# envoy/ksql

Measured on AMD Instinct MI355X. Metric: records/sec, windowed GROUP BY (COUNT(*) TUMBLING 5 s GROUP BY card_number HAVING > 3), higher is better.
Workload: dtype int64

## Files before the change

### ksql_amd/csrc/khip_agg_c1.hip

```cpp
#include <algorithm>
#include <cstdio>
#include <type_traits>
#include <vector>

#include "khip_part.hpp"

namespace khip {

constexpr int C1_TILE = 65536;
constexpr int C1_NT = 512;
constexpr int C1_CH = 8192;
template <class T>
__device__ __forceinline__ T c1_ld(const T* p) {
  return *p;
}
constexpr int C1_SEGMAX = 512;
constexpr int C1_SEGB = 7;
constexpr int C1_SEGOF = 512;
constexpr uint32_t C1_SENT = 0x80000000u;

__device__ __forceinline__ int bits_of(uint64_t v) { return v ? 64 - __clzll((long long)v) : 0; }

__device__ __forceinline__ int64_t ci_ld(const int64_t* ci, int k) {
  const uint64_t v = (uint64_t)__hip_atomic_load(&ci[k], __ATOMIC_RELAXED, __HIP_MEMORY_SCOPE_AGENT);
// ... 295 lines not shown
    ts4[3] = t_ok ? 1 : 0;
  }
}

__global__ __launch_bounds__(256) void k_c1_krange(const int64_t* __restrict__ keys, int64_t stride, int64_t n,
                                                   long long* __restrict__ out) {
  int64_t mx = INT64_MIN, mxn = INT64_MIN;
  for (int64_t i = blockIdx.x * (int64_t)blockDim.x + threadIdx.x; i < n; i += (int64_t)gridDim.x * blockDim.x) {
    const int64_t k = keys[i * stride];
    mx = k > mx ? k : mx;
    mxn = ~k > mxn ? ~k : mxn;
  }
  for (int off = 32; off > 0; off >>= 1) {
    const int64_t a = __shfl_xor(mx, off, 64), b = __shfl_xor(mxn, off, 64);
    mx = a > mx ? a : mx;
    mxn = b > mxn ? b : mxn;
  }
  if ((threadIdx.x & 63) == 0) {
    atomicMax(&out[0], (long long)mxn);
    atomicMax(&out[1], (long long)mx);
  }
}

__global__ __launch_bounds__(1024) void k_c1_runpos(const uint32_t* __restrict__ ttot, int64_t nT,
                                                    uint32_t* __restrict__ tbase) {
  __shared__ uint32_t wsum[16];
  const int lane = threadIdx.x & 63, wave = threadIdx.x >> 6;
  const uint32_t* in = ttot + (int64_t)blockIdx.x * nT;
  uint32_t* out = tbase + (int64_t)blockIdx.x * (nT + 1);
  uint32_t carry = 0u;
  for (int64_t t0 = 0; t0 < nT; t0 += 1024) {
    const int64_t t = t0 + threadIdx.x;
    const uint32_t c = t < nT ? in[t] : 0u;
    uint32_t incl = c;
    for (int off = 1; off < 64; off <<= 1) {
      const uint32_t y = __shfl_up(incl, off, 64);
      if (lane >= off) incl += y;
    }
    if (lane == 63) wsum[wave] = incl;
    __syncthreads();
    uint32_t before = 0u, tot = 0u;
#pragma unroll
    for (int k = 0; k < 16; k++) {
      before += k < wave ? wsum[k] : 0u;
      tot += wsum[k];
    }
    if (t < nT) out[t] = carry + before + incl - c;
    carry += tot;
    __syncthreads();
  }
  if (threadIdx.x == 0) out[nT] = carry;
}

__global__ __launch_bounds__(256) void k_c1_chunks(const int* __restrict__ cstart, int B,
                                                   const uint32_t* __restrict__ tbase, const uint16_t* __restrict__ rloc,
                                                   int64_t nT, int sh, int ch, const int64_t* __restrict__ ci,
                                                   uint32_t* __restrict__ cinfo) {
  if (ci_ld(ci, CI_GATE) == 0) return;
  const int w = blockIdx.x * blockDim.x + threadIdx.x;
  if (w >= (int)ci_ld(ci, CI_NCHUNK)) return;
  int a = 0, e = B;
  while (e - a > 1) {
    const int m = (a + e) >> 1;
    if (cstart[m] <= w) a = m;
    else e = m;
  }
  const int b = a;
  const int64_t nSt = nT << sh, spt = (int64_t)1 << sh;
  const uint32_t* tb = tbase + (int64_t)b * (nT + 1);
  const uint16_t* rl = rloc + (int64_t)b * nSt;
  const int64_t lo = (int64_t)(w - cstart[b]) * ch, blen = (int64_t)tb[nT];
  const int64_t hi = blen - lo < ch ? blen : lo + ch;
  int64_t t0 = 0, e0 = nT, t1 = 0, e1 = nT;
  while (e0 - t0 > 1 || e1 - t1 > 1) {
    const int64_t m0 = (t0 + e0) >> 1, m1 = (t1 + e1) >> 1;
    const int64_t p0 = (int64_t)tb[m0], p1 = (int64_t)tb[m1];
    if (e0 - t0 > 1) {
      if (p0 <= lo) t0 = m0;
      else e0 = m0;
    }
    if (e1 - t1 > 1) {
      if (p1 < hi) t1 = m1;
      else e1 = m1;
    }
  }
  const int64_t b0 = (int64_t)tb[t0], b1 = (int64_t)tb[t1];
  int64_t sa = t0 << sh, sl = t1 << sh;
  for (int64_t half = spt >> 1; half > 0; half >>= 1) {
    const int64_t q0 = b0 + (int64_t)rl[sa + half], q1 = b1 + (int64_t)rl[sl + half];
    if (q0 <= lo) sa += half;
    if (q1 < hi) sl += half;
  }
  cinfo[2 * w] = (uint32_t)sa;
  cinfo[2 * w + 1] = (uint32_t)(sl + 1 - sa);
}

__device__ __forceinline__ void chunk_map(const uint32_t* __restrict__ tb, const uint16_t* __restrict__ rl,
                                          const uint16_t* __restrict__ ro, int64_t nSt, int sh,
                                          const uint32_t* __restrict__ cinfo, int w, int64_t S, int64_t lo, int len,
                                          uint32_t* map) {
  const int64_t s0 = cinfo[2 * w];
  const int R = (int)cinfo[2 * w + 1];
  for (int k = threadIdx.x; k < R; k += blockDim.x) {
    const int64_t s = s0 + k, p = run_pos(tb, rl, nSt, sh, s), pe = run_pos(tb, rl, nSt, sh, s + 1);
    const int64_t a = p > lo ? p : lo, e = pe < lo + len ? pe : lo + len;
    const uint32_t src = (uint32_t)(s * S + (int64_t)ro[s] + (a - p));
    for (int64_t x = a; x < e; x++) map[x - lo] = src + (uint32_t)(x - a);
  }
  __syncthreads();
}

__global__ __launch_bounds__(1024) void k_c1_check(
    const int64_t* __restrict__ tilestat, const int64_t* __restrict__ tpart, int64_t nT, int64_t size, int64_t adv,
    FastDiv fd, int64_t grace, int64_t close0, int fresh, int log2B, int log2P, int wide, int ch, int kbmax, int pbits,
    const uint32_t* __restrict__ tbase, int64_t* __restrict__ bb, int* __restrict__ cstart,
    int64_t* __restrict__ ci, int64_t* __restrict__ stream_time, int64_t* __restrict__ res,
    unsigned long long* __restrict__ ctr, unsigned long long* __restrict__ closed_ctr, unsigned long long closed_n) {
  __shared__ int64_t wmx[16];
  __shared__ int64_t red[2][16];
  __shared__ unsigned long long lsum[T_NPART];
  __shared__ int lslow;
  __shared__ int64_t wtot[8];
  __shared__ int wnch[8], wmxc[8];
  const int lane = threadIdx.x & 63, wave = threadIdx.x >> 6;
  if (threadIdx.x == 0) lslow = 0;
  if (threadIdx.x < T_NPART) lsum[threadIdx.x] = 0ULL;
  const int B = 1 << log2B;
  const uint32_t btot = (int)threadIdx.x < B ? tbase[(int64_t)threadIdx.x * (nT + 1) + nT] : 0u;
  const int64_t st0 = *stream_time;
  const int64_t K = (nT + 1023) / 1024;
  const int64_t g0 = threadIdx.x * K, g1 = g0 + K < nT ? g0 + K : nT;
  int64_t m = -1;
  for (int64_t g = g0; g < g1; g++) m = tilestat[4 * g] > m ? tilestat[4 * g] : m;
  const int64_t incl = wave_incl_max(m);
  if (lane == 63) wmx[wave] = incl;
  __syncthreads();
  int64_t pre = st0;
  for (int w = 0; w < wave; w++) pre = wmx[w] > pre ? wmx[w] : pre;
  const int64_t excl = __shfl_up(incl, 1, 64);
  int64_t run = lane == 0 ? pre : (excl > pre ? excl : pre);
  int64_t gmn = INT64_MAX, gmx = -1;
  int64_t tsum[T_NPART] = {};
  bool slow = false;
  for (int64_t g = g0; g < g1; g++) {
    const int64_t* t4 = tilestat + 4 * g;
    const int64_t mx = t4[0], mn = t4[1];
    if (mn != INT64_MAX) {
      slow |= t4[3] == 0 || run > t4[2];
      gmn = mn < gmn ? mn : gmn;
    }
    run = mx > run ? mx : run;
    gmx = mx > gmx ? mx : gmx;
#pragma unroll
    for (int k = 0; k < T_NPART; k++) tsum[k] += tpart[g * T_NPART + k];
  }
  if (slow) lslow = 1;
  for (int off = 32; off > 0; off >>= 1) {
    const int64_t a = __shfl_xor(gmn, off, 64), b = __shfl_xor(gmx, off, 64);
    gmn = a < gmn ? a : gmn;
    gmx = b > gmx ? b : gmx;
  }
#pragma unroll
// ... 60 lines not shown
           (int)lslow, mxc, (long)kmin, (long)kmax, (long)gmn, (long)gmx, (long)ci[CI_T0], (long)st0, (long)nT);
#endif
  const uint64_t krange = kmax >= kmin ? (uint64_t)kmax - (uint64_t)kmin : 0;
  const bool fits = !wide && !kfail && krange < ((1ULL << kbmax) - 1);
  const int64_t kb = ci_ld(ci, CI_KBASE);
  ci[CI_FITS] = fits ? 1 : 0;
  ci[CI_REASON] = ok && !wide && kfail ? 2 : (ok && !wide && !fits ? 1 : 0);
  ci[CI_KMINC] = kmin;
  ci[CI_KSHIFT] = (int64_t)((uint64_t)kmin - (uint64_t)kb);
  ok = ok && (wide || fits);
  int64_t lo = INT64_MAX, hi = INT64_MIN;
  if (gmx >= 0) {
    const int64_t l = gmn - size + adv;
    lo = (int64_t)fast_udiv((uint64_t)(l > 0 ? l : 0), fd);
    hi = (int64_t)fast_udiv((uint64_t)gmx, fd);
  }
  if (!fresh) {
    int64_t rlo = res[0];
    const int64_t rhi = res[1];
    if (close0 != INT64_MIN && rlo != INT64_MAX) {
      const int64_t c = close0 - size;
      const int64_t lb = c >= 0 ? (int64_t)fast_udiv((uint64_t)c, fd) + 1 : 0;
      rlo = rlo > lb ? rlo : lb;
    }
    lo = rlo < lo ? rlo : lo;
    hi = rhi > hi ? rhi : hi;
  }
  const bool none = lo > hi;
  if (none) lo = hi = 0;
  ok = ok && (uint64_t)(hi - lo) < (wide ? ((uint64_t)1 << log2P) - 1 : (pbits ? 0x7FFFFFFEull : 0xFFFFFFFEull));
  const int wbits = bits_of((uint64_t)(hi - lo)), kbits = bits_of(krange);
  ci[CI_GATE] = ok ? 1 : 0;
  if (!ok) return;
  ci[CI_WBASE] = lo;
  ci[CI_WHI] = hi - lo;
  ci[CI_WBITS] = wbits;
  ci[CI_KBITS] = kbits;
  ci[CI_KRANGE] = (int64_t)krange;
  ci[CI_ID32] = !wide && kbits + wbits + pbits <= 31 ? 1 : 0;
  ci[CI_WIDE] = wide;
  ci[CI_TMIN] = gmx >= 0 ? gmn : 0;
  ci[CI_TMAX] = gmx;
  ci[CI_NCHUNK] = acc;
  *stream_time = gmx > st0 ? gmx : st0;
  res[0] = none ? INT64_MAX : lo;
  res[1] = none ? INT64_MIN : hi;
  ctr[CTR_ADDED] = ctr[CTR_FAILED] = ctr[CTR_NEED] = 0ULL;
  for (int k = 0; k < T_NPART; k++) ctr[CTR_TILE + k] = lsum[k];
  if (closed_ctr) *closed_ctr = closed_n;
}

template <int U, int NT, bool WIDE>
__global__ __launch_bounds__(NT) __attribute__((amdgpu_waves_per_eu(4))) void k_c1_refine(
    const uint64_t* __restrict__ srcA, const int64_t* __restrict__ bb, const int* __restrict__ cstart, int log2B,
    int log2P, int fbits, uint64_t* __restrict__ srec, uint16_t* __restrict__ seg, const int64_t* __restrict__ ci,
    const uint32_t* __restrict__ srcAT, uint32_t* __restrict__ srecT, const uint32_t* __restrict__ tbase,
    const uint16_t* __restrict__ rloc, const uint16_t* __restrict__ roff, int64_t nT, int sh, int64_t S,
    const uint32_t* __restrict__ cinfo) {
  if (ci_ld(ci, CI_GATE) == 0) return;
  const int w = blockIdx.x;
  if (w >= (int)ci_ld(ci, CI_NCHUNK)) return;
  extern __shared__ __attribute__((aligned(16))) char smem[];
  __shared__ int lb, lnv;
  __shared__ int wsum[NT / 64];
  static_assert(U * NT == C1_CH, "refine chunk");
  const int F = 1 << fbits, B = 1 << log2B;
  uint32_t* cnt = (uint32_t*)smem;
  uint32_t* sbase = cnt + F;
  uint64_t* stage = (uint64_t*)(smem + (size_t)F * 8);
  for (int f = threadIdx.x; f < F; f += NT) cnt[f] = 0u;
  if (threadIdx.x == 0) lb = -1;
  __syncthreads();
  for (int b = threadIdx.x; b < B; b += NT)
    if (cstart[b] <= w && w < cstart[b + 1]) lb = b;
  __syncthreads();
  const int b = lb;
  if (b < 0) return;
  const int64_t lo = bb[b] + (int64_t)(w - cstart[b]) * C1_CH;
  const int64_t bend = bb[b + 1];
  const int len = (int)(bend - lo < C1_CH ? bend - lo : C1_CH);
  const int64_t kmin = ci_ld(ci, CI_KMINC);
  const uint64_t kshift = WIDE ? 0 : (uint64_t)ci_ld(ci, CI_KSHIFT) << 32;
  const int shift = 64 - log2P;
  const int64_t nSt = nT << sh;
  chunk_map(tbase + (int64_t)b * (nT + 1), rloc + (int64_t)b * nSt, roff + (int64_t)b * nSt, nSt, sh, cinfo, w, S,
            lo - bb[b], len, (uint32_t*)stage);
  uint64_t r[U];
  uint32_t f[U], rank[U], t32[U];
#pragma unroll
  for (int u = 0; u < U; u++) {
    const int j = threadIdx.x + u * NT;
    const uint32_t src = ((const uint32_t*)stage)[j < len ? j : len - 1];
    r[u] = c1_ld(srcA + src) - kshift;
    if constexpr (WIDE) t32[u] = c1_ld(srcAT + src);
  }
#pragma unroll
  for (int u = 0; u < U; u++) {
    const int j = threadIdx.x + u * NT;
    const bool v = j < len && (WIDE ? t32[u] : (uint32_t)r[u]) != C1_SENT;
    f[u] = WIDE ? (uint32_t)(r[u] >> shift) & (uint32_t)(F - 1)
                : (uint32_t)(key_hash(kmin + (int64_t)(r[u] >> 32)) >> shift) & (uint32_t)(F - 1);
    rank[u] = v ? atomicAdd(&cnt[f[u]], 1u) : 0xFFFFFFFFu;
  }
  __syncthreads();
  {
    const int t = threadIdx.x, lane = t & 63, wave = t >> 6;
    const uint32_t c = t < F ? cnt[t] : 0u;
    uint32_t incl = c;
    for (int off = 1; off < 64; off <<= 1) {
      const uint32_t y = __shfl_up(incl, off, 64);
      if (lane >= off) incl += y;
    }
    if (lane == 63) wsum[wave] = (int)incl;
    __syncthreads();
    uint32_t before = 0, tot = 0;
#pragma unroll
    for (int k = 0; k < NT / 64; k++) {
      before += k < wave ? (uint32_t)wsum[k] : 0u;
      tot += (uint32_t)wsum[k];
    }
    if (t < F) {
      sbase[t] = before + incl - c;
      seg[(int64_t)w * (F + 1) + t] = (uint16_t)(before + incl - c);
    }
    if (t == 0) {
      seg[(int64_t)w * (F + 1) + F] = (uint16_t)tot;
      lnv = (int)tot;
    }
  }
  __syncthreads();
  const int nv = lnv;
#pragma unroll
  for (int u = 0; u < U; u++)
    if (rank[u] != 0xFFFFFFFFu) stage[sbase[f[u]] + rank[u]] = r[u];
  __syncthreads();
  for (int j = threadIdx.x; j < nv; j += NT) srec[lo + j] = stage[j];
  if constexpr (WIDE) {
    __syncthreads();
    uint32_t* stage32 = (uint32_t*)stage;
#pragma unroll
    for (int u = 0; u < U; u++)
      if (rank[u] != 0xFFFFFFFFu) stage32[sbase[f[u]] + rank[u]] = t32[u];
    __syncthreads();
    for (int j = threadIdx.x; j < nv; j += NT) srecT[lo + j] = stage32[j];
  }
}

#ifdef KHIP_TUNING
#define C1M_T(k)                                                                        \
  do {                                                                                  \
    if (dbg && threadIdx.x == 0) {                                                      \
      const unsigned long long now_ = wall_clock64();                                   \
      atomicAdd(&dbg[(k)], now_ - t_last);                                              \
      t_last = now_;                                                                    \
    }                                                                                   \
  } while (0)
#define C1M_T0 unsigned long long t_last = dbg ? wall_clock64() : 0ULL
#else
#define C1M_T(k) \
  do {           \
  } while (0)
#define C1M_T0 (void)dbg
#endif

struct C1Q {
  int32_t log2P, fbits, log2H, sw, hv_active, hv_op, hmax;
  int64_t size, adv, cmax, hv_i64;
  FastDiv fd;
  FastDiv32 fd32;
  uint8_t* chg;
};

__device__ __forceinline__ bool c1q_having(const C1Q& q, uint64_t c) {
  const int64_t v = (int64_t)c;
  switch (q.hv_op) {
    case KHIP_OP_GT: return v > q.hv_i64;
    case KHIP_OP_GE: return v >= q.hv_i64;
    case KHIP_OP_LT: return v < q.hv_i64;
    case KHIP_OP_LE: return v <= q.hv_i64;
    case KHIP_OP_EQ: return v == q.hv_i64;
    case KHIP_OP_NE: return v != q.hv_i64;
  }
  return true;
}

template <class ID>
__device__ __forceinline__ uint32_t c1_hash(ID id) {
  if constexpr (sizeof(ID) == 4) return (uint32_t)id * 0x9E3779B1u;
  else return ((uint32_t)id * 0x9E3779B1u) ^ ((uint32_t)(id >> 32) * 0x85EBCA77u);
}
__device__ __forceinline__ uint32_t c1_sub(uint32_t h, int sbits) {
  h ^= h >> 15;
  h *= 0x2C1B3C6Du;
  return (h >> 12) & ((1u << sbits) - 1u);
}

template <class ID>
__device__ __forceinline__ int c1_find_id(const KLDS ID* ids, ID id, uint32_t e, int H) {
// ... 828 lines not shown
    uint32_t t32u[U];
    const uint32_t tot = stage_step_runs<U, NT, ulonglong2, false>(rec, t32u, bin, ok, B, cnt, sbase, wsum, sp, nullptr,
                                                                   srec, nullptr, t * SPT + st, lrc + st * B,
                                                                   lro + st * B);
    step_krange<NT, ulonglong2>(sp, tot, 0x7FFFFFFFu, lkr);
    for (int off = 32; off > 0; off >>= 1) {
      const int a = __shfl_xor(tmx, off, 64), b = __shfl_xor(tmn, off, 64);
      tmx = a > tmx ? a : tmx;
      tmn = b < tmn ? b : tmn;
    }
    if ((threadIdx.x & 63) == 0 && tmx != INT32_MIN) {
      atomicMax(&lt[st & 1][0], tmx);
      atomicMin(&lt[st & 1][1], tmn);
    }
    if (threadIdx.x == 0 && st > 0) publish(s0 - S, st - 1);
  }
  flush_run_counts<SPT, NT>(lrc, lro, B, st_last, t, nT, rloc, roff, ttot);
  if (kor) lkfail = 1;
  __syncthreads();
  if (threadIdx.x == 0 && s0 > base) publish(s0 - S, st_last);
  if (threadIdx.x == 0) run_krange(lkr, lkfail, kb, ci);
  c_acc = wave_sum(c_acc);
  c_nk = wave_sum(c_nk);
  c_nr = wave_sum(c_nr);
  c_bt = wave_sum(c_bt);
  c_app = wave_sum(c_app);
  if ((threadIdx.x & 63) == 0) {
    if (c_acc) atomicAdd(&lc[0], (unsigned long long)c_acc);
    if (c_nk) atomicAdd(&lc[1], (unsigned long long)c_nk);
    if (c_nr) atomicAdd(&lc[2], (unsigned long long)c_nr);
    if (c_bt) atomicAdd(&lc[3], (unsigned long long)c_bt);
    if (c_app) atomicAdd(&lc[4], (unsigned long long)c_app);
  }
  __syncthreads();
  if (threadIdx.x == 0) {
    int64_t* tp = tpart + t * T_NPART;
    tp[T_ACCEPTED] = (int64_t)lc[0];
    tp[T_NULL_KEY] = (int64_t)lc[1];
    tp[T_NULL_ROW] = (int64_t)lc[2];
    tp[T_BAD_TS] = (int64_t)lc[3];
    tp[T_APPLIED] = hop ? (int64_t)lc[4] : (int64_t)lc[0];
    tp[T_LATE] = 0;
    if (lfail) atomicOr((unsigned long long*)&ci[CI_TFAIL], 1ULL);
    int64_t* ts4 = tilestat + t * 4;
    ts4[0] = t_rmax;
    ts4[1] = t_min;
    ts4[2] = t_bound;
    ts4[3] = t_ok ? 1 : 0;
  }
}

template <int U, int NT>
__global__ __launch_bounds__(NT) __attribute__((amdgpu_waves_per_eu(4))) void k_c1v_refine(
    const ulonglong2* __restrict__ srcA, const int64_t* __restrict__ bb, const int* __restrict__ cstart, int log2B,
    int log2P, int fbits, ulonglong2* __restrict__ srec, uint16_t* __restrict__ seg, const int64_t* __restrict__ ci,
    const uint32_t* __restrict__ tbase, const uint16_t* __restrict__ rloc, const uint16_t* __restrict__ roff,
    int64_t nT, int sh, int64_t S, const uint32_t* __restrict__ cinfo) {
  if (ci_ld(ci, CI_GATE) == 0) return;
  const int w = blockIdx.x;
  if (w >= (int)ci_ld(ci, CI_NCHUNK)) return;
  extern __shared__ __attribute__((aligned(16))) char smem[];
  __shared__ int lb, lnv;
  __shared__ int wsum[NT / 64];
  constexpr int CH = U * NT;
  static_assert(CH == C1V_CH, "refine chunk");
  const int F = 1 << fbits, B = 1 << log2B;
  uint32_t* cnt = (uint32_t*)smem;
  uint32_t* sbase = cnt + F;
  ulonglong2* stage = (ulonglong2*)(smem + (((size_t)F * 8 + 15) & ~(size_t)15));
  for (int f = threadIdx.x; f < F; f += NT) cnt[f] = 0u;
  if (threadIdx.x == 0) lb = -1;
  __syncthreads();
  for (int b = threadIdx.x; b < B; b += NT)
    if (cstart[b] <= w && w < cstart[b + 1]) lb = b;
  __syncthreads();
  const int b = lb;
  if (b < 0) return;
  const int64_t lo = bb[b] + (int64_t)(w - cstart[b]) * CH;
  const int64_t bend = bb[b + 1];
  const int len = (int)(bend - lo < CH ? bend - lo : CH);
  const int64_t kmin = ci_ld(ci, CI_KMINC);
  const uint64_t kshift = (uint64_t)ci_ld(ci, CI_KSHIFT) << 32;
  const int shift = 64 - log2P;
  const int64_t nSt = nT << sh;
  chunk_map(tbase + (int64_t)b * (nT + 1), rloc + (int64_t)b * nSt, roff + (int64_t)b * nSt, nSt, sh, cinfo, w, S,
            lo - bb[b], len, (uint32_t*)stage);
  ulonglong2 r[U];
  uint32_t f[U], rank[U];
#pragma unroll
  for (int u = 0; u < U; u++) {
    const int j = threadIdx.x + u * NT;
    const uint32_t src = ((const uint32_t*)stage)[j < len ? j : len - 1];
    r[u] = ld_nt2(srcA + src);
    r[u].x -= kshift;
  }
#pragma unroll
  for (int u = 0; u < U; u++) {
    const int j = threadIdx.x + u * NT;
    const bool v = j < len && (uint32_t)r[u].x != C1_SENT;
    f[u] = (uint32_t)(key_hash(kmin + (int64_t)((r[u].x >> 32) & 0x7FFFFFFFull)) >> shift) & (uint32_t)(F - 1);
    rank[u] = v ? atomicAdd(&cnt[f[u]], 1u) : 0xFFFFFFFFu;
  }
  __syncthreads();
  {
    const int t = threadIdx.x, lane = t & 63, wave = t >> 6;
    const uint32_t c = t < F ? cnt[t] : 0u;
    uint32_t incl = c;
    for (int off = 1; off < 64; off <<= 1) {
      const uint32_t y = __shfl_up(incl, off, 64);
      if (lane >= off) incl += y;
    }
    if (lane == 63) wsum[wave] = (int)incl;
    __syncthreads();
    uint32_t before = 0, tot = 0;
#pragma unroll
    for (int k = 0; k < NT / 64; k++) {
      before += k < wave ? (uint32_t)wsum[k] : 0u;
      tot += (uint32_t)wsum[k];
    }
    if (t < F) {
      sbase[t] = before + incl - c;
      seg[(int64_t)w * (F + 1) + t] = (uint16_t)(before + incl - c);
    }
    if (t == 0) {
      seg[(int64_t)w * (F + 1) + F] = (uint16_t)tot;
      lnv = (int)tot;
    }
  }
  __syncthreads();
  const int nv = lnv;
#pragma unroll
  for (int u = 0; u < U; u++)
    if (rank[u] != 0xFFFFFFFFu) stage[sbase[f[u]] + rank[u]] = r[u];
  __syncthreads();
  for (int j = threadIdx.x; j < nv; j += NT) srec[lo + j] = stage[j];
}

struct C1VQ {
  int32_t log2P, fbits, log2H, sw, hmax, f64, fan;
  int32_t off_sum, off_min, off_max, off_rt, off_star, off_cnt, off_list, off_spre;
  int32_t word_op[C1V_MAXW];
  int64_t size, adv, cmax;
  FastDiv fd;
  FastDiv32 fd32;
  uint64_t init[C1V_MAXW];
  HavingDev having;
  uint8_t* chg;
};

template <class T>
__device__ __forceinline__ KLDS T* c1v_plane(char* smem, int off) {
  return (KLDS T*)((KLDS char*)smem + off);
}

constexpr int PM_STAR = 1, PM_CNT = 2, PM_SUM = 4, PM_MIN = 8, PM_MAX = 16, PM_F64 = 32, PM_SPEC = 64;
constexpr int PM_C5 = PM_SPEC | PM_SUM;
constexpr int PM_C3 = PM_SPEC | PM_CNT | PM_SUM | PM_MIN | PM_MAX | PM_F64;
template <int PM>
struct C1VP {
  const C1VQ& q;
  __device__ __forceinline__ bool star() const { return PM ? (PM & PM_STAR) != 0 : q.off_star >= 0; }
  __device__ __forceinline__ bool cnt() const { return PM ? (PM & PM_CNT) != 0 : q.off_cnt >= 0; }
  __device__ __forceinline__ bool sum() const { return PM ? (PM & PM_SUM) != 0 : q.off_sum >= 0; }
  __device__ __forceinline__ bool mn() const { return PM ? (PM & PM_MIN) != 0 : q.off_min >= 0; }
  __device__ __forceinline__ bool mx() const { return PM ? (PM & PM_MAX) != 0 : q.off_max >= 0; }
  __device__ __forceinline__ bool f64() const { return PM ? (PM & PM_F64) != 0 : q.f64 != 0; }
};

template <int PM>
__device__ __forceinline__ uint64_t c1v_word(const C1VQ& q, char* smem, int e, int k, uint64_t w) {
  const C1VP<PM> v{q};
  switch (q.word_op[k]) {
    case OP_INC: return v.star() ? w + c1v_plane<uint32_t>(smem, q.off_star)[e] : w;
    case OP_INC_VALID: return v.cnt() ? w + c1v_plane<uint32_t>(smem, q.off_cnt)[e] : w;
    case OP_ADD_I64: return v.sum() && !v.f64() ? w + c1v_plane<uint64_t>(smem, q.off_sum)[e] : w;
    case OP_ADD_F64:
      if (v.sum() && v.f64()) {
        double a, b = c1v_plane<double>(smem, q.off_sum)[e];
        __builtin_memcpy(&a, &w, 8);
        a += b;
        __builtin_memcpy(&w, &a, 8);
      }
      return w;
    case OP_MIN:
      if (v.mn()) {
        const int64_t m = c1v_plane<int64_t>(smem, q.off_min)[e];
        if (m < (int64_t)w) w = (uint64_t)m;
      }
// ... 834 lines not shown
  g->adv = a->desc.advance_ms;
  g->fd = make_fastdiv(g->adv);
  g->close0 = a->host_stream_time >= 0 ? a->host_stream_time - a->grace : INT64_MIN;
  g->wide = !g->val && s.c1_wide;
  g->srecAT = (uint32_t*)(s.srecA.as<uint64_t>() + n + 1);
  g->srecT = (uint32_t*)(s.srec.as<uint64_t>() + n + 1);
  g->tt = s.c1rc.as<uint32_t>();
  g->tb = s.c1rp.as<uint32_t>();
  g->rl = s.c1rl.as<uint16_t>();
  g->ro = s.c1ro.as<uint16_t>();
  return KHIP_OK;
}

static khip_status c1_scatter(khip_agg* a, const C1In& in, const C1Geo& g) {
  PartState& s = a->part;
  ev_record_part(a, 0);
  const int has_kb = s.c1_kb_valid ? 1 : 0;
  const int64_t* st_at = in.st_at;
  if (g.val) {
    constexpr int UV = C1V_UV;
    const RowsIn* rows = in.rows;
    const C1VCol vc{rows ? nullptr : in.cols->data[in.vcol], rows ? nullptr : in.cols->valid[in.vcol],
                    a->ap.col_type[in.vcol]};
    const RowsIn ri = rows ? *rows : RowsIn{};
    auto sk = rows ? (st_at ? k_c1v_scatter<UV, C1_NT, true, true> : k_c1v_scatter<UV, C1_NT, false, true>)
                   : (st_at ? k_c1v_scatter<UV, C1_NT, true, false> : k_c1v_scatter<UV, C1_NT, false, false>);
    const size_t lds = run_stage_lds(g.B, UV * C1_NT, 16, false) + run_cnt_lds(g.B, C1_TILE / (UV * C1_NT));
    if (lds > 64 * 1024) hipFuncSetAttribute((const void*)sk, hipFuncAttributeMaxDynamicSharedMemorySize, (int)lds);
    hipLaunchKernelGGL(sk, dim3(g.nT), dim3(C1_NT), lds, a->stream, in.keys, in.ts, in.kv, in.rv, vc, ri, g.n, g.nT,
                       g.log2B, g.rl, g.ro, g.tt, (ulonglong2*)s.srecA.p, s.tilemax.as<int64_t>(),
                       s.tpart.as<int64_t>(), g.ci, st_at, a->desc.size_ms, g.adv, g.fd,
                       a->desc.size_ms != g.adv ? 1 : 0, a->grace, (const int64_t*)a->stream_time.as<int64_t>(),
                       s.c1_kbase, has_kb);
  } else {
    constexpr int U = 8;
    auto sk = g.wide ? (st_at ? k_c1_scatter<U, C1_NT, true, true> : k_c1_scatter<U, C1_NT, true, false>)
                     : (st_at ? k_c1_scatter<U, C1_NT, false, true> : k_c1_scatter<U, C1_NT, false, false>);
    const size_t lds = run_stage_lds(g.B, U * C1_NT, 8, g.wide) + run_cnt_lds(g.B, C1_TILE / (U * C1_NT));
    if (lds > 64 * 1024) hipFuncSetAttribute((const void*)sk, hipFuncAttributeMaxDynamicSharedMemorySize, (int)lds);
    hipLaunchKernelGGL(sk, dim3(g.nT), dim3(C1_NT), lds, a->stream, in.keys, in.ts, in.kv, in.rv, g.n, g.nT, g.log2B,
                       g.rl, g.ro, g.tt, s.srecA.as<uint64_t>(), s.tilemax.as<int64_t>(), s.tpart.as<int64_t>(), g.ci,
                       st_at, g.srecAT, a->desc.size_ms, g.adv, g.fd, a->grace,
                       (const int64_t*)a->stream_time.as<int64_t>(), s.c1_kbase, has_kb);
  }
  KHIP_TRY_HIP(hipGetLastError());
  hipLaunchKernelGGL(k_c1_runpos, dim3(g.B), dim3(1024), 0, a->stream, (const uint32_t*)g.tt, g.nT, g.tb);
  KHIP_TRY_HIP(hipGetLastError());
  ev_record_part(a, 1);
  return KHIP_OK;
}

static khip_status c1_refine(khip_agg* a, const C1Geo& g) {
  PartState& s = a->part;
  if (g.val) {
    auto rk = k_c1v_refine<C1V_CH / C1_NT, C1_NT>;
    const size_t lds = (((size_t)g.F * 8 + 15) & ~(size_t)15) + (size_t)C1V_CH * 16;
    hipFuncSetAttribute((const void*)rk, hipFuncAttributeMaxDynamicSharedMemorySize, (int)lds);
    hipLaunchKernelGGL(rk, dim3((unsigned)g.nchunk_max), dim3(C1_NT), lds, a->stream, (const ulonglong2*)s.srecA.p,
                       s.c1bb.as<int64_t>(), g.cstart, g.log2B, s.log2P, g.fbits, (ulonglong2*)s.srec.p, g.seg, g.ci,
                       (const uint32_t*)g.tb, (const uint16_t*)g.rl, (const uint16_t*)g.ro, g.nT, g.sh, g.S,
                       (const uint32_t*)s.c1ci.as<uint32_t>());
  } else {
    constexpr int U = C1_CH / C1_NT;
    auto rk = g.wide ? k_c1_refine<U, C1_NT, true> : k_c1_refine<U, C1_NT, false>;
    const size_t lds = (size_t)g.F * 8 + (size_t)C1_CH * 8;
    if (lds > 64 * 1024) hipFuncSetAttribute((const void*)rk, hipFuncAttributeMaxDynamicSharedMemorySize, (int)lds);
    hipLaunchKernelGGL(rk, dim3((unsigned)g.nchunk_max), dim3(C1_NT), lds, a->stream, s.srecA.as<uint64_t>(),
                       s.c1bb.as<int64_t>(), g.cstart, g.log2B, s.log2P, g.fbits, s.srec.as<uint64_t>(), g.seg, g.ci,
                       (const uint32_t*)g.srecAT, g.srecT, (const uint32_t*)g.tb, (const uint16_t*)g.rl,
                       (const uint16_t*)g.ro, g.nT, g.sh, g.S, (const uint32_t*)s.c1ci.as<uint32_t>());
  }
  KHIP_TRY_HIP(hipGetLastError());
  return KHIP_OK;
}

static khip_status c1_records(khip_agg* a, const C1In& in, const C1Geo& g) {
  PartState& s = a->part;
  KHIP_TRY(c1_scatter(a, in, g));
  hipLaunchKernelGGL(k_c1_check, dim3(1), dim3(1024), 0, a->stream, s.tilemax.as<int64_t>(),
                     (const int64_t*)s.tpart.as<int64_t>(), g.nT, a->desc.size_ms, g.adv, g.fd, a->grace, g.close0,
                     s.res_fresh ? 1 : 0, g.log2B, s.log2P, g.wide ? 1 : 0, g.CH, g.val ? 31 : 32, g.panes ? 1 : 0,
                     (const uint32_t*)g.tb, s.c1bb.as<int64_t>(), g.cstart, g.ci, a->stream_time.as<int64_t>(),
                     s.res.as<int64_t>(), s.ctr.as<unsigned long long>(), s.closed_ctr.as<unsigned long long>(),
                     (unsigned long long)s.closed_n);
  KHIP_TRY(s.c1ci.ensure((size_t)g.nchunk_max * 8));
  hipLaunchKernelGGL(k_c1_chunks, dim3((unsigned)ceil_div(g.nchunk_max, 256)), dim3(256), 0, a->stream,
                     (const int*)g.cstart, g.B, (const uint32_t*)g.tb, (const uint16_t*)g.rl, g.nT, g.sh, g.CH,
                     (const int64_t*)g.ci, s.c1ci.as<uint32_t>());
  KHIP_TRY(c1_refine(a, g));
  ev_record_part(a, 2);
  return KHIP_OK;
}

static C1Q c1_make_q(khip_agg* a, const C1Geo& g, int log2H) {
  C1Q cq{};
  cq.log2P = a->part.log2P;
  cq.fbits = g.fbits;
  cq.log2H = log2H;
  cq.sw = a->sw;
  cq.hv_active = a->having.active;
  cq.hv_op = a->having.op;
  cq.hv_i64 = a->having.i64;
  cq.hmax = (int)((int64_t)(1 << log2H) * 3 / 4);
  cq.size = a->desc.size_ms;
  cq.adv = g.adv;
  cq.fd = g.fd;
  cq.fd32 = make_fastdiv32((uint32_t)g.adv);
  return cq;
}

static void c1v_make_q(khip_agg* a, const C1Geo& g, int vcol, C1Merge* m) {
  C1VQ& vq0 = m->vq0;
  m->v_log2H = 12;
  while (m->v_log2H > 9 && c1v_layout(a, m->v_log2H, 4, g.log2B, &vq0) > C1V_LDS2) m->v_log2H--;
  m->v_log2H = (int)knob("KHIP_C1V_LOG2H", m->v_log2H);

  vq0.log2P = a->part.log2P;
  vq0.fbits = g.fbits;
  vq0.log2H = m->v_log2H;
  vq0.sw = a->sw;
  vq0.hmax = (int)((int64_t)(1 << m->v_log2H) * 3 / 4);
  vq0.fan = (int)(a->desc.size_ms / g.adv);
  vq0.f64 = 0;
  for (int k = 0; k < C1V_MAXW; k++) {
    vq0.word_op[k] = -1;
    vq0.init[k] = (uint64_t)a->init.w[k];
  }
  for (int o = 0; o < a->ap.n_ops; o++) {
    vq0.word_op[a->ap.ops[o].word] = a->ap.ops[o].kind;
    if (a->ap.ops[o].kind == OP_ADD_F64) vq0.f64 = 1;
  }
  if (a->ap.col_type[vcol] == KHIP_TYPE_DOUBLE) vq0.f64 = 1;
  int pm = 0;
  for (int o = 0; o < a->ap.n_ops; o++) {
    const int k = a->ap.ops[o].kind;
    pm |= k == OP_INC ? PM_STAR : k == OP_INC_VALID ? PM_CNT : k == OP_MIN ? PM_MIN : k == OP_MAX ? PM_MAX : PM_SUM;
  }
  pm |= PM_SPEC | (vq0.f64 ? PM_F64 : 0);
  m->v_pm = ((pm != PM_C5 && pm != PM_C3) || knob("KHIP_C1V_SPEC", 1) == 0) ? 0 : pm;
  vq0.size = a->desc.size_ms;
  vq0.adv = g.adv;
// ... 192 lines not shown
```

Baseline: 59.50 billion.

## Precompute per-chunk descriptors and pipeline refine with next-chunk run prefetch

k_c1_chunks now writes a full 32-byte chunk descriptor (bucket, offsets, run range), so refine blocks no longer scan cstart over all buckets and then resolve runs with run_pos binary searches. Refine is unified into one templated routine that prefetches the next chunk's run bounds while sorting the current one, and can loop over chunks with a grid stride. Ranks and bins are packed into one register, and output is written directly from registers through bounds-clamped buffer stores instead of a strided copy-out loop. The cost is a larger descriptor buffer, more registers per thread, and more complex code. Since the grid still equals nchunk_max, the next-chunk path rarely runs.

```diff
diff --git a/ksql_amd/csrc/khip_agg_c1.hip b/ksql_amd/csrc/khip_agg_c1.hip
--- a/ksql_amd/csrc/khip_agg_c1.hip
+++ b/ksql_amd/csrc/khip_agg_c1.hip
@@ -371,13 +371,20 @@
   if (threadIdx.x == 0) out[nT] = carry;
 }
 
+struct alignas(32) C1Chunk {
+  uint32_t b, len, lo, lrel, s0, R, pad[2];
+};
+
 __global__ __launch_bounds__(256) void k_c1_chunks(const int* __restrict__ cstart, int B,
                                                    const uint32_t* __restrict__ tbase, const uint16_t* __restrict__ rloc,
                                                    int64_t nT, int sh, int ch, const int64_t* __restrict__ ci,
-                                                   uint32_t* __restrict__ cinfo) {
-  if (ci_ld(ci, CI_GATE) == 0) return;
+                                                   const int64_t* __restrict__ bb, int nmax, C1Chunk* __restrict__ cd) {
   const int w = blockIdx.x * blockDim.x + threadIdx.x;
-  if (w >= (int)ci_ld(ci, CI_NCHUNK)) return;
+  if (w >= nmax) return;
+  if (ci_ld(ci, CI_GATE) == 0 || w >= (int)ci_ld(ci, CI_NCHUNK)) {
+    cd[w] = C1Chunk{};
+    return;
+  }
   int a = 0, e = B;
   while (e - a > 1) {
     const int m = (a + e) >> 1;
@@ -410,23 +417,226 @@
     if (q0 <= lo) sa += half;
     if (q1 < hi) sl += half;
   }
-  cinfo[2 * w] = (uint32_t)sa;
-  cinfo[2 * w + 1] = (uint32_t)(sl + 1 - sa);
-}
-
-__device__ __forceinline__ void chunk_map(const uint32_t* __restrict__ tb, const uint16_t* __restrict__ rl,
-                                          const uint16_t* __restrict__ ro, int64_t nSt, int sh,
-                                          const uint32_t* __restrict__ cinfo, int w, int64_t S, int64_t lo, int len,
+  C1Chunk c{};
+  c.b = (uint32_t)b;
+  c.len = (uint32_t)(hi - lo);
+  c.lo = (uint32_t)(bb[b] + lo);
+  c.lrel = (uint32_t)lo;
+  c.s0 = (uint32_t)sa;
+  c.R = (uint32_t)(sl + 1 - sa);
+  cd[w] = c;
+}
+
+
+struct C1Run {
+  uint32_t a, al, b, bl, ro;
+  __device__ __forceinline__ uint32_t p() const { return a + al; }
+  __device__ __forceinline__ uint32_t pe(bool last) const { return b + (last ? 0u : bl); }
+};
+
+struct C1RunTab {
+  const uint32_t* tb;
+  const uint16_t *rl, *ro;
+  int64_t nSt;
+  int sh;
+};
+
+__device__ __forceinline__ C1RunTab run_tab(const uint32_t* __restrict__ tbase, const uint16_t* __restrict__ rloc,
+                                            const uint16_t* __restrict__ roff, int64_t nT, int sh, uint32_t b) {
+  const int64_t nSt = nT << sh;
+  return C1RunTab{tbase + (int64_t)b * (nT + 1), rloc + (int64_t)b * nSt, roff + (int64_t)b * nSt, nSt, sh};
+}
+
+__device__ __forceinline__ C1Run run_ld(const C1RunTab& rt, const C1Chunk& d, int k) {
+  const int64_t s = (int64_t)d.s0 + (k < (int)d.R ? k : 0);
+  const int64_t s1 = s + 1 < rt.nSt ? s + 1 : s;
+  return C1Run{rt.tb[s >> rt.sh], rt.rl[s], rt.tb[(s + 1) >> rt.sh], rt.rl[s1], rt.ro[s]};
+}
+
+template <int NT>
+__device__ __forceinline__ void chunk_map(const C1RunTab& rt, const C1Chunk& d, const C1Run& pre, int64_t S,
                                           uint32_t* map) {
-  const int64_t s0 = cinfo[2 * w];
-  const int R = (int)cinfo[2 * w + 1];
-  for (int k = threadIdx.x; k < R; k += blockDim.x) {
-    const int64_t s = s0 + k, p = run_pos(tb, rl, nSt, sh, s), pe = run_pos(tb, rl, nSt, sh, s + 1);
-    const int64_t a = p > lo ? p : lo, e = pe < lo + len ? pe : lo + len;
-    const uint32_t src = (uint32_t)(s * S + (int64_t)ro[s] + (a - p));
-    for (int64_t x = a; x < e; x++) map[x - lo] = src + (uint32_t)(x - a);
-  }
-  __syncthreads();
+  const uint32_t lo = d.lrel, hi = d.lrel + d.len;
+  auto fill = [&](int k, const C1Run& r) {
+    const uint32_t p = r.p(), pe = r.pe((int64_t)d.s0 + k + 1 >= rt.nSt);
+    const uint32_t a = p > lo ? p : lo, e = pe < hi ? pe : hi;
+    const uint32_t src = (uint32_t)(((int64_t)d.s0 + k) * S) + r.ro + (a - p);
+    for (uint32_t x = a; x < e; x++) map[x - lo] = src + (x - a);
+  };
+  if ((int)threadIdx.x < (int)d.R) fill(threadIdx.x, pre);
+  for (int k = threadIdx.x + NT; k < (int)d.R; k += NT) fill(k, run_ld(rt, d, k));
+}
+
+__device__ __forceinline__ C1Chunk chunk_ld(const C1Chunk* __restrict__ cd, int w, int nmax) {
+  C1Chunk d{};
+  if (w < nmax) d = cd[w];
+  return d;
+}
+
+typedef uint32_t c1_u32x2 __attribute__((ext_vector_type(2)));
+typedef uint32_t c1_u32x4 __attribute__((ext_vector_type(4)));
+typedef uint64_t c1_u64x2 __attribute__((ext_vector_type(2)));
+
+__device__ __forceinline__ __amdgpu_buffer_rsrc_t out_rsrc(void* base, uint32_t bytes) {
+  return __builtin_amdgcn_make_buffer_rsrc(base, (short)0, (int)bytes, 0x00020000);
+}
+__device__ __forceinline__ void out_st(__amdgpu_buffer_rsrc_t rs, uint32_t j, uint32_t v) {
+  __builtin_amdgcn_raw_buffer_store_b32(v, rs, (int)(j * 4u), 0, 0);
+}
+__device__ __forceinline__ void out_st(__amdgpu_buffer_rsrc_t rs, uint32_t j, uint64_t v) {
+  const c1_u32x2 d = {(uint32_t)v, (uint32_t)(v >> 32)};
+  __builtin_amdgcn_raw_buffer_store_b64(d, rs, (int)(j * 8u), 0, 0);
+}
+__device__ __forceinline__ void out_st(__amdgpu_buffer_rsrc_t rs, uint32_t j, ulonglong2 v) {
+  const c1_u32x4 d = {(uint32_t)v.x, (uint32_t)(v.x >> 32), (uint32_t)v.y, (uint32_t)(v.y >> 32)};
+  __builtin_amdgcn_raw_buffer_store_b128(d, rs, (int)(j * 16u), 0, 0);
+}
+
+__device__ __forceinline__ uint64_t rec_ld(const uint64_t* p) { return c1_ld(p); }
+__device__ __forceinline__ ulonglong2 rec_ld(const ulonglong2* p) {
+  const c1_u64x2 v = c1_ld((const c1_u64x2*)p);
+  return make_ulonglong2(v.x, v.y);
+}
+__device__ __forceinline__ uint64_t rec_w0(uint64_t r) { return r; }
+__device__ __forceinline__ uint64_t rec_w0(const ulonglong2& r) { return (uint64_t)r.x; }
+__device__ __forceinline__ void rec_rebase(uint64_t& r, uint64_t k) { r -= k; }
+__device__ __forceinline__ void rec_rebase(ulonglong2& r, uint64_t k) { r.x -= k; }
+
+template <class R, int U, int NT, bool WIDE>
+__device__ __forceinline__ void refine_store(const R (&o)[U], const uint32_t (&oT)[WIDE ? U : 1], R* __restrict__ srec,
+                                             uint32_t* __restrict__ srecT, uint32_t lo, uint32_t nv) {
+  const __amdgpu_buffer_rsrc_t rs = out_rsrc(srec + lo, nv * (uint32_t)sizeof(R));
+#pragma unroll
+  for (int u = 0; u < U; u++) out_st(rs, threadIdx.x + u * NT, o[u]);
+  if constexpr (WIDE) {
+    const __amdgpu_buffer_rsrc_t rt = out_rsrc(srecT + lo, nv * 4u);
+#pragma unroll
+    for (int u = 0; u < U; u++) out_st(rt, threadIdx.x + u * NT, oT[u]);
+  }
+}
+
+template <class R, int U, int NT, bool WIDE>
+__device__ __forceinline__ void refine_chunks(const R* __restrict__ srcA, R* __restrict__ srec,
+                                              const uint32_t* __restrict__ srcAT, uint32_t* __restrict__ srecT,
+                                              uint16_t* __restrict__ seg, const int64_t* __restrict__ ci,
+                                              const uint32_t* __restrict__ tbase, const uint16_t* __restrict__ rloc,
+                                              const uint16_t* __restrict__ roff, int64_t nT, int sh, int64_t S,
+                                              const C1Chunk* __restrict__ cd, int nmax, int log2P, int fbits,
+                                              char* smem) {
+  constexpr bool VAL = sizeof(R) == 16;
+  constexpr int UT = WIDE ? U : 1;
+  static_assert(U * NT <= 8192, "a rank fits 13 bits, a position a u16");
+  __shared__ int lnv;
+  __shared__ int wsum[NT / 64];
+  const int t_wg = threadIdx.x, t = t_wg;
+  const int F = 1 << fbits, shift = 64 - log2P;
+  uint32_t* cnt = (uint32_t*)smem;
+  uint32_t* sbase = cnt + F;
+  R* stage = (R*)(smem + (((size_t)F * 8 + 15) & ~(size_t)15));
+  uint32_t* map = (uint32_t*)stage;
+  int w = blockIdx.x;
+  C1Chunk d = chunk_ld(cd, w, nmax);
+  if (d.len == 0) return;
+  const int64_t kmin = ci_ld(ci, CI_KMINC);
+  const uint64_t kshift = WIDE ? 0 : (uint64_t)ci_ld(ci, CI_KSHIFT) << 32;
+  for (int f = t; f < F; f += NT) cnt[f] = 0u;
+
+  auto load_chunk = [&](const C1Chunk& c, R(&r)[U], uint32_t(&t32)[UT]) {
+#pragma unroll
+    for (int u = 0; u < U; u++) {
+      const uint32_t j = t + u * NT;
+      const uint32_t src = map[j < c.len ? j : c.len - 1];
+      r[u] = rec_ld(srcA + src);
+      if constexpr (WIDE) t32[u] = c1_ld(srcAT + src);
+      if (u % 4 == 3) __builtin_amdgcn_sched_barrier(0);
+    }
+  };
+  auto sort_chunk = [&](const C1Chunk& c, int cw, R(&r)[U], const uint32_t(&t32)[UT], R(&o)[U],
+                        uint32_t(&oT)[UT]) -> uint32_t {
+    int t = t_wg;
+    asm volatile("" : "+v"(t));
+    const int lane = t & 63, wave = t >> 6;
+    uint32_t pk[U];
+#pragma unroll
+    for (int u = 0; u < U; u++) {
+      const uint32_t j = t + u * NT;
+      rec_rebase(r[u], kshift);
+      const uint64_t w0 = rec_w0(r[u]);
+      const bool v = j < c.len && (WIDE ? t32[u] : (uint32_t)w0) != C1_SENT;
+      const uint32_t f =
+          WIDE ? (uint32_t)(w0 >> shift) & (uint32_t)(F - 1)
+               : (uint32_t)(key_hash(kmin + (int64_t)(VAL ? (w0 >> 32) & 0x7FFFFFFFull : w0 >> 32)) >> shift) &
+                     (uint32_t)(F - 1);
+      pk[u] = v ? atomicAdd(&cnt[f], 1u) << 8 | f : 0xFFFFFFFFu;
+    }
+    lds_barrier();
+    {
+      const uint32_t n = t < F ? cnt[t] : 0u;
+      uint32_t incl = n;
+      for (int off = 1; off < 64; off <<= 1) {
+        const uint32_t y = __shfl_up(incl, off, 64);
+        if (lane >= off) incl += y;
+      }
+      if (lane == 63) wsum[wave] = (int)incl;
+      lds_barrier();
+      uint32_t before = 0, tot = 0;
+#pragma unroll
+      for (int k = 0; k < NT / 64; k++) {
+        before += k < wave ? (uint32_t)wsum[k] : 0u;
+        tot += (uint32_t)wsum[k];
+      }
+      if (t < F) {
+        sbase[t] = before + incl - n;
+        cnt[t] = 0u;
+        seg[(int64_t)cw * (F + 1) + t] = (uint16_t)(before + incl - n);
+      }
+      if (t == 0) {
+        seg[(int64_t)cw * (F + 1) + F] = (uint16_t)tot;
+        lnv = (int)tot;
+      }
+    }
+    lds_barrier();
+#pragma unroll
+    for (int u = 0; u < U; u++)
+      if (pk[u] != 0xFFFFFFFFu) stage[sbase[pk[u] & 255u] + (pk[u] >> 8)] = r[u];
+    lds_barrier();
+    const uint32_t nv = (uint32_t)__builtin_amdgcn_readfirstlane(lnv);
+#pragma unroll
+    for (int u = 0; u < U; u++) o[u] = stage[t + u * NT];
+    if constexpr (WIDE) {
+      uint32_t* stage32 = (uint32_t*)stage;
+      lds_barrier();
+#pragma unroll
+      for (int u = 0; u < U; u++)
+        if (pk[u] != 0xFFFFFFFFu) stage32[sbase[pk[u] & 255u] + (pk[u] >> 8)] = t32[u];
+      lds_barrier();
+#pragma unroll
+      for (int u = 0; u < U; u++) oT[u] = stage32[t + u * NT];
+    }
+    return nv;
+  };
+
+  C1RunTab rt = run_tab(tbase, rloc, roff, nT, sh, d.b);
+  C1Run pre = run_ld(rt, d, t);
+  R r[U], o[U];
+  uint32_t t32[UT], oT[UT];
+  for (;;) {
+    lds_barrier();
+    chunk_map<NT>(rt, d, pre, S, map);
+    lds_barrier();
+    load_chunk(d, r, t32);
+    const int wn = w + (int)gridDim.x;
+    const C1Chunk dn = chunk_ld(cd, wn, nmax);
+    if (dn.len) {
+      rt = run_tab(tbase, rloc, roff, nT, sh, dn.b);
+      pre = run_ld(rt, dn, t);
+    }
+    const uint32_t nv = sort_chunk(d, w, r, t32, o, oT);
+    refine_store<R, U, NT, WIDE>(o, oT, srec, srecT, d.lo, nv);
+    if (dn.len == 0) break;
+    d = dn;
+    w = wn;
+  }
 }
 
 __global__ __launch_bounds__(1024) void k_c1_check(
@@ -593,98 +803,14 @@
 
 template <int U, int NT, bool WIDE>
 __global__ __launch_bounds__(NT) __attribute__((amdgpu_waves_per_eu(4))) void k_c1_refine(
-    const uint64_t* __restrict__ srcA, const int64_t* __restrict__ bb, const int* __restrict__ cstart, int log2B,
-    int log2P, int fbits, uint64_t* __restrict__ srec, uint16_t* __restrict__ seg, const int64_t* __restrict__ ci,
-    const uint32_t* __restrict__ srcAT, uint32_t* __restrict__ srecT, const uint32_t* __restrict__ tbase,
-    const uint16_t* __restrict__ rloc, const uint16_t* __restrict__ roff, int64_t nT, int sh, int64_t S,
-    const uint32_t* __restrict__ cinfo) {
-  if (ci_ld(ci, CI_GATE) == 0) return;
-  const int w = blockIdx.x;
-  if (w >= (int)ci_ld(ci, CI_NCHUNK)) return;
+    const uint64_t* __restrict__ srcA, int log2P, int fbits, uint64_t* __restrict__ srec, uint16_t* __restrict__ seg,
+    const int64_t* __restrict__ ci, const uint32_t* __restrict__ srcAT, uint32_t* __restrict__ srecT,
+    const uint32_t* __restrict__ tbase, const uint16_t* __restrict__ rloc, const uint16_t* __restrict__ roff,
+    int64_t nT, int sh, int64_t S, const C1Chunk* __restrict__ cd, int nmax) {
   extern __shared__ __attribute__((aligned(16))) char smem[];
-  __shared__ int lb, lnv;
-  __shared__ int wsum[NT / 64];
   static_assert(U * NT == C1_CH, "refine chunk");
-  const int F = 1 << fbits, B = 1 << log2B;
-  uint32_t* cnt = (uint32_t*)smem;
-  uint32_t* sbase = cnt + F;
-  uint64_t* stage = (uint64_t*)(smem + (size_t)F * 8);
-  for (int f = threadIdx.x; f < F; f += NT) cnt[f] = 0u;
-  if (threadIdx.x == 0) lb = -1;
-  __syncthreads();
-  for (int b = threadIdx.x; b < B; b += NT)
-    if (cstart[b] <= w && w < cstart[b + 1]) lb = b;
-  __syncthreads();
-  const int b = lb;
-  if (b < 0) return;
-  const int64_t lo = bb[b] + (int64_t)(w - cstart[b]) * C1_CH;
-  const int64_t bend = bb[b + 1];
-  const int len = (int)(bend - lo < C1_CH ? bend - lo : C1_CH);
-  const int64_t kmin = ci_ld(ci, CI_KMINC);
-  const uint64_t kshift = WIDE ? 0 : (uint64_t)ci_ld(ci, CI_KSHIFT) << 32;
-  const int shift = 64 - log2P;
-  const int64_t nSt = nT << sh;
-  chunk_map(tbase + (int64_t)b * (nT + 1), rloc + (int64_t)b * nSt, roff + (int64_t)b * nSt, nSt, sh, cinfo, w, S,
-            lo - bb[b], len, (uint32_t*)stage);
-  uint64_t r[U];
-  uint32_t f[U], rank[U], t32[U];
-#pragma unroll
-  for (int u = 0; u < U; u++) {
-    const int j = threadIdx.x + u * NT;
-    const uint32_t src = ((const uint32_t*)stage)[j < len ? j : len - 1];
-    r[u] = c1_ld(srcA + src) - kshift;
-    if constexpr (WIDE) t32[u] = c1_ld(srcAT + src);
-  }
-#pragma unroll
-  for (int u = 0; u < U; u++) {
-    const int j = threadIdx.x + u * NT;
-    const bool v = j < len && (WIDE ? t32[u] : (uint32_t)r[u]) != C1_SENT;
-    f[u] = WIDE ? (uint32_t)(r[u] >> shift) & (uint32_t)(F - 1)
-                : (uint32_t)(key_hash(kmin + (int64_t)(r[u] >> 32)) >> shift) & (uint32_t)(F - 1);
-    rank[u] = v ? atomicAdd(&cnt[f[u]], 1u) : 0xFFFFFFFFu;
-  }
-  __syncthreads();
-  {
-    const int t = threadIdx.x, lane = t & 63, wave = t >> 6;
-    const uint32_t c = t < F ? cnt[t] : 0u;
-    uint32_t incl = c;
-    for (int off = 1; off < 64; off <<= 1) {
-      const uint32_t y = __shfl_up(incl, off, 64);
-      if (lane >= off) incl += y;
-    }
-    if (lane == 63) wsum[wave] = (int)incl;
-    __syncthreads();
-    uint32_t before = 0, tot = 0;
-#pragma unroll
-    for (int k = 0; k < NT / 64; k++) {
-      before += k < wave ? (uint32_t)wsum[k] : 0u;
-      tot += (uint32_t)wsum[k];
-    }
-    if (t < F) {
-      sbase[t] = before + incl - c;
-      seg[(int64_t)w * (F + 1) + t] = (uint16_t)(before + incl - c);
-    }
-    if (t == 0) {
-      seg[(int64_t)w * (F + 1) + F] = (uint16_t)tot;
-      lnv = (int)tot;
-    }
-  }
-  __syncthreads();
-  const int nv = lnv;
-#pragma unroll
-  for (int u = 0; u < U; u++)
-    if (rank[u] != 0xFFFFFFFFu) stage[sbase[f[u]] + rank[u]] = r[u];
-  __syncthreads();
-  for (int j = threadIdx.x; j < nv; j += NT) srec[lo + j] = stage[j];
-  if constexpr (WIDE) {
-    __syncthreads();
-    uint32_t* stage32 = (uint32_t*)stage;
-#pragma unroll
-    for (int u = 0; u < U; u++)
-      if (rank[u] != 0xFFFFFFFFu) stage32[sbase[f[u]] + rank[u]] = t32[u];
-    __syncthreads();
-    for (int j = threadIdx.x; j < nv; j += NT) srecT[lo + j] = stage32[j];
-  }
+  refine_chunks<uint64_t, U, NT, WIDE>(srcA, srec, srcAT, srecT, seg, ci, tbase, rloc, roff, nT, sh, S, cd, nmax, log2P,
+                                       fbits, smem);
 }
 
 #ifdef KHIP_TUNING
@@ -1619,88 +1745,14 @@
 
 template <int U, int NT>
 __global__ __launch_bounds__(NT) __attribute__((amdgpu_waves_per_eu(4))) void k_c1v_refine(
-    const ulonglong2* __restrict__ srcA, const int64_t* __restrict__ bb, const int* __restrict__ cstart, int log2B,
-    int log2P, int fbits, ulonglong2* __restrict__ srec, uint16_t* __restrict__ seg, const int64_t* __restrict__ ci,
-    const uint32_t* __restrict__ tbase, const uint16_t* __restrict__ rloc, const uint16_t* __restrict__ roff,
-    int64_t nT, int sh, int64_t S, const uint32_t* __restrict__ cinfo) {
-  if (ci_ld(ci, CI_GATE) == 0) return;
-  const int w = blockIdx.x;
-  if (w >= (int)ci_ld(ci, CI_NCHUNK)) return;
+    const ulonglong2* __restrict__ srcA, int log2P, int fbits, ulonglong2* __restrict__ srec,
+    uint16_t* __restrict__ seg, const int64_t* __restrict__ ci, const uint32_t* __restrict__ tbase,
+    const uint16_t* __restrict__ rloc, const uint16_t* __restrict__ roff, int64_t nT, int sh, int64_t S,
+    const C1Chunk* __restrict__ cd, int nmax) {
   extern __shared__ __attribute__((aligned(16))) char smem[];
-  __shared__ int lb, lnv;
-  __shared__ int wsum[NT / 64];
-  constexpr int CH = U * NT;
-  static_assert(CH == C1V_CH, "refine chunk");
-  const int F = 1 << fbits, B = 1 << log2B;
-  uint32_t* cnt = (uint32_t*)smem;
-  uint32_t* sbase = cnt + F;
-  ulonglong2* stage = (ulonglong2*)(smem + (((size_t)F * 8 + 15) & ~(size_t)15));
-  for (int f = threadIdx.x; f < F; f += NT) cnt[f] = 0u;
-  if (threadIdx.x == 0) lb = -1;
-  __syncthreads();
-  for (int b = threadIdx.x; b < B; b += NT)
-    if (cstart[b] <= w && w < cstart[b + 1]) lb = b;
-  __syncthreads();
-  const int b = lb;
-  if (b < 0) return;
-  const int64_t lo = bb[b] + (int64_t)(w - cstart[b]) * CH;
-  const int64_t bend = bb[b + 1];
-  const int len = (int)(bend - lo < CH ? bend - lo : CH);
-  const int64_t kmin = ci_ld(ci, CI_KMINC);
-  const uint64_t kshift = (uint64_t)ci_ld(ci, CI_KSHIFT) << 32;
-  const int shift = 64 - log2P;
-  const int64_t nSt = nT << sh;
-  chunk_map(tbase + (int64_t)b * (nT + 1), rloc + (int64_t)b * nSt, roff + (int64_t)b * nSt, nSt, sh, cinfo, w, S,
-            lo - bb[b], len, (uint32_t*)stage);
-  ulonglong2 r[U];
-  uint32_t f[U], rank[U];
-#pragma unroll
-  for (int u = 0; u < U; u++) {
-    const int j = threadIdx.x + u * NT;
-    const uint32_t src = ((const uint32_t*)stage)[j < len ? j : len - 1];
-    r[u] = ld_nt2(srcA + src);
-    r[u].x -= kshift;
-  }
-#pragma unroll
-  for (int u = 0; u < U; u++) {
-    const int j = threadIdx.x + u * NT;
-    const bool v = j < len && (uint32_t)r[u].x != C1_SENT;
-    f[u] = (uint32_t)(key_hash(kmin + (int64_t)((r[u].x >> 32) & 0x7FFFFFFFull)) >> shift) & (uint32_t)(F - 1);
-    rank[u] = v ? atomicAdd(&cnt[f[u]], 1u) : 0xFFFFFFFFu;
-  }
-  __syncthreads();
-  {
-    const int t = threadIdx.x, lane = t & 63, wave = t >> 6;
-    const uint32_t c = t < F ? cnt[t] : 0u;
-    uint32_t incl = c;
-    for (int off = 1; off < 64; off <<= 1) {
-      const uint32_t y = __shfl_up(incl, off, 64);
-      if (lane >= off) incl += y;
-    }
-    if (lane == 63) wsum[wave] = (int)incl;
-    __syncthreads();
-    uint32_t before = 0, tot = 0;
-#pragma unroll
-    for (int k = 0; k < NT / 64; k++) {
-      before += k < wave ? (uint32_t)wsum[k] : 0u;
-      tot += (uint32_t)wsum[k];
-    }
-    if (t < F) {
-      sbase[t] = before + incl - c;
-      seg[(int64_t)w * (F + 1) + t] = (uint16_t)(before + incl - c);
-    }
-    if (t == 0) {
-      seg[(int64_t)w * (F + 1) + F] = (uint16_t)tot;
-      lnv = (int)tot;
-    }
-  }
-  __syncthreads();
-  const int nv = lnv;
-#pragma unroll
-  for (int u = 0; u < U; u++)
-    if (rank[u] != 0xFFFFFFFFu) stage[sbase[f[u]] + rank[u]] = r[u];
-  __syncthreads();
-  for (int j = threadIdx.x; j < nv; j += NT) srec[lo + j] = stage[j];
+  static_assert(U * NT == C1V_CH, "refine chunk");
+  refine_chunks<ulonglong2, U, NT, false>(srcA, srec, nullptr, nullptr, seg, ci, tbase, rloc, roff, nT, sh, S, cd, nmax,
+                                          log2P, fbits, smem);
 }
 
 struct C1VQ {
@@ -2641,23 +2693,23 @@
 
 static khip_status c1_refine(khip_agg* a, const C1Geo& g) {
   PartState& s = a->part;
+  const unsigned grid = (unsigned)g.nchunk_max;
+  const C1Chunk* cd = (const C1Chunk*)s.c1ci.p;
   if (g.val) {
     auto rk = k_c1v_refine<C1V_CH / C1_NT, C1_NT>;
     const size_t lds = (((size_t)g.F * 8 + 15) & ~(size_t)15) + (size_t)C1V_CH * 16;
     hipFuncSetAttribute((const void*)rk, hipFuncAttributeMaxDynamicSharedMemorySize, (int)lds);
-    hipLaunchKernelGGL(rk, dim3((unsigned)g.nchunk_max), dim3(C1_NT), lds, a->stream, (const ulonglong2*)s.srecA.p,
-                       s.c1bb.as<int64_t>(), g.cstart, g.log2B, s.log2P, g.fbits, (ulonglong2*)s.srec.p, g.seg, g.ci,
-                       (const uint32_t*)g.tb, (const uint16_t*)g.rl, (const uint16_t*)g.ro, g.nT, g.sh, g.S,
-                       (const uint32_t*)s.c1ci.as<uint32_t>());
+    hipLaunchKernelGGL(rk, dim3(grid), dim3(C1_NT), lds, a->stream, (const ulonglong2*)s.srecA.p, s.log2P, g.fbits,
+                       (ulonglong2*)s.srec.p, g.seg, (const int64_t*)g.ci, (const uint32_t*)g.tb,
+                       (const uint16_t*)g.rl, (const uint16_t*)g.ro, g.nT, g.sh, g.S, cd, (int)g.nchunk_max);
   } else {
     constexpr int U = C1_CH / C1_NT;
     auto rk = g.wide ? k_c1_refine<U, C1_NT, true> : k_c1_refine<U, C1_NT, false>;
-    const size_t lds = (size_t)g.F * 8 + (size_t)C1_CH * 8;
+    const size_t lds = (((size_t)g.F * 8 + 15) & ~(size_t)15) + (size_t)C1_CH * 8;
     if (lds > 64 * 1024) hipFuncSetAttribute((const void*)rk, hipFuncAttributeMaxDynamicSharedMemorySize, (int)lds);
-    hipLaunchKernelGGL(rk, dim3((unsigned)g.nchunk_max), dim3(C1_NT), lds, a->stream, s.srecA.as<uint64_t>(),
-                       s.c1bb.as<int64_t>(), g.cstart, g.log2B, s.log2P, g.fbits, s.srec.as<uint64_t>(), g.seg, g.ci,
-                       (const uint32_t*)g.srecAT, g.srecT, (const uint32_t*)g.tb, (const uint16_t*)g.rl,
-                       (const uint16_t*)g.ro, g.nT, g.sh, g.S, (const uint32_t*)s.c1ci.as<uint32_t>());
+    hipLaunchKernelGGL(rk, dim3(grid), dim3(C1_NT), lds, a->stream, (const uint64_t*)s.srecA.as<uint64_t>(), s.log2P,
+                       g.fbits, s.srec.as<uint64_t>(), g.seg, (const int64_t*)g.ci, (const uint32_t*)g.srecAT, g.srecT,
+                       (const uint32_t*)g.tb, (const uint16_t*)g.rl, (const uint16_t*)g.ro, g.nT, g.sh, g.S, cd, (int)g.nchunk_max);
   }
   KHIP_TRY_HIP(hipGetLastError());
   return KHIP_OK;
@@ -2672,10 +2724,11 @@
                      (const uint32_t*)g.tb, s.c1bb.as<int64_t>(), g.cstart, g.ci, a->stream_time.as<int64_t>(),
                      s.res.as<int64_t>(), s.ctr.as<unsigned long long>(), s.closed_ctr.as<unsigned long long>(),
                      (unsigned long long)s.closed_n);
-  KHIP_TRY(s.c1ci.ensure((size_t)g.nchunk_max * 8));
+  KHIP_TRY(s.c1ci.ensure((size_t)g.nchunk_max * sizeof(C1Chunk)));
   hipLaunchKernelGGL(k_c1_chunks, dim3((unsigned)ceil_div(g.nchunk_max, 256)), dim3(256), 0, a->stream,
                      (const int*)g.cstart, g.B, (const uint32_t*)g.tb, (const uint16_t*)g.rl, g.nT, g.sh, g.CH,
-                     (const int64_t*)g.ci, s.c1ci.as<uint32_t>());
+                     (const int64_t*)g.ci, (const int64_t*)s.c1bb.as<int64_t>(), (int)g.nchunk_max,
+                     (C1Chunk*)s.c1ci.p);
   KHIP_TRY(c1_refine(a, g));
   ev_record_part(a, 2);
   return KHIP_OK;
```

Result: no change. 60.06 billion, median of 6 (+0.9%).
